# zcablii/SM3Det

Hardware: NVIDIA H100
Metric: backbone images/sec @1024^2 (fwd+bwd) (higher is better)
Workload: dtype f32 (bf16 hi+lo split operands on wgmma, fp32 accumulate; SIMT fp32 elsewhere)

## Files before the change

sm3det_b200/csrc/gemm_tc.cu:

```cuda
#define SM3_GEMM_KERNEL_IMPL
#include "gemm_tc.cuh"
#include <mutex>

namespace sm3 {
const char* last_error();
namespace gemm {

int pick_bn(int N) {
  static const int cand[] = {128, 96, 64, 32};
  for (int bn : cand)
    if (N % bn == 0) return bn;
  return 0;
}

static bool aligned16(const void* p) { return (reinterpret_cast<uintptr_t>(p) & 15u) == 0; }

long long packed_elems(int N, int K) {
  const long long kblocks = (K + BK - 1) / BK;
  return (long long)N * kblocks * BK * 2;
}

__global__ void __launch_bounds__(256) pack_b_kernel(const float* __restrict__ B, long long s_mn, long long s_k,
                                                    long long group_stride, int N, int K, int BN, uint16_t* __restrict__ out,
                                                    long long chunks_per_group) {
  const long long i = (long long)blockIdx.x * blockDim.x + threadIdx.x;
  if (i >= chunks_per_group) return;
  const int g = blockIdx.y;
  const int kblocks = (K + BK - 1) / BK;
  const int n = (int)(i % N);
  const long long r = i / N;
  const int c = (int)(r % 4), kb = (int)(r / 4);
  const float* src = B + (long long)g * group_stride + (long long)n * s_mn;
  uint32_t hi[4], lo[4];
#pragma unroll
  for (int e = 0; e < 8; e += 2) {
    float v[2];
#pragma unroll
    for (int q = 0; q < 2; ++q) {
      const int k = kb * BK + c * 8 + e + q;
      v[q] = (k < K) ? __ldg(src + (long long)k * s_k) : 0.f;
    }
    const uint32_t u0 = __float_as_uint(v[0]), u1 = __float_as_uint(v[1]);
    hi[e / 2] = __byte_perm(u0, u1, 0x7632);
    const uint32_t r0 = __float_as_uint(v[0] - __uint_as_float(u0 & 0xFFFF0000u)) + 0x8000u;
    const uint32_t r1 = __float_as_uint(v[1] - __uint_as_float(u1 & 0xFFFF0000u)) + 0x8000u;
    lo[e / 2] = __byte_perm(r0, r1, 0x7632);
  }
  const int nt = n / BN, row = n % BN;
  uint8_t* tile = reinterpret_cast<uint8_t*>(out + (long long)g * ((long long)N * kblocks * BK * 2)) +
                  ((long long)nt * kblocks + kb) * ((long long)BN * 128);
  const uint32_t o = kmajor_sw64_offset((uint32_t)row, (uint32_t)c);
  *reinterpret_cast<uint4*>(tile + o) = make_uint4(hi[0], hi[1], hi[2], hi[3]);
  *reinterpret_cast<uint4*>(tile + (long long)BN * 64 + o) = make_uint4(lo[0], lo[1], lo[2], lo[3]);
}

int pack_b(const float* B, long long s_mn, long long s_k, long long group_stride, int groups, int N, int K,
           uint16_t* out, cudaStream_t stream, int tile) {
  SM3_REQUIRE(B && out && N > 0 && K > 0 && groups >= 1, SM3_ERR_INVALID_ARG, "gemm pack: bad argument");
  const int BN = tile > 0 ? tile : pick_bn(N);
  SM3_REQUIRE(BN > 0 && BN % 8 == 0 && BN <= 256 && N % BN == 0, SM3_ERR_UNSUPPORTED_SHAPE, "gemm pack: N=%d has no tile width (tile=%d)", N, tile);
  SM3_REQUIRE((reinterpret_cast<uintptr_t>(out) & 15u) == 0, SM3_ERR_INVALID_ARG, "gemm pack: output must be 16B aligned");
  const long long kblocks = (K + BK - 1) / BK;
  const long long chunks = (long long)N * kblocks * 4;
  dim3 grid((unsigned)((chunks + 255) / 256), (unsigned)groups);
  pack_b_kernel<<<grid, 256, 0, stream>>>(B, s_mn, s_k, group_stride, N, K, BN, out, chunks);
  return check_launch("pack_b_kernel");
}

long long packed_act_elems(long long rows, int cols, int mn_major, int tile) {
  if (!mn_major) {
    const long long rt = (rows + tile - 1) / tile, kb = (cols + BK - 1) / BK;
    return rt * kb * 2 * (long long)tile * BK;
  }
  const long long ct = (cols + tile - 1) / tile, kb = (rows + BK - 1) / BK;
  return ct * kb * 2 * (long long)(plane_bytes(tile, true) / 2);
}

__global__ void __launch_bounds__(256) pack_act_k_kernel(const float* __restrict__ X, long long ld, const int* __restrict__ row_index,
                                                        long long rows, int K, int tile, uint16_t* __restrict__ out,
                                                        long long chunks) {
  const long long i = (long long)blockIdx.x * blockDim.x + threadIdx.x;
  if (i >= chunks) return;
  const int kblocks = (K + BK - 1) / BK;
  const int cpr = kblocks * 4;
  const long long row = i / cpr;
  const int cc = (int)(i % cpr), kb = cc >> 2, c = cc & 3;
  long long src_row = row < rows ? row : -1;
  if (src_row >= 0 && row_index) src_row = __ldg(row_index + row);
  float v[8];
#pragma unroll
  for (int e = 0; e < 8; ++e) v[e] = 0.f;
  if (src_row >= 0) {
    const int k = kb * BK + c * 8;
    const float* src = X + src_row * ld + k;
    if (k + 8 <= K) { const float4 a = ldg_f4(src), b = ldg_f4(src + 4); v[0] = a.x; v[1] = a.y; v[2] = a.z; v[3] = a.w; v[4] = b.x; v[5] = b.y; v[6] = b.z; v[7] = b.w; }
    else { for (int e = 0; e < 8; ++e) if (k + e < K) v[e] = __ldg(src + e); }
  }
  uint32_t hi[4], lo[4];
#pragma unroll
  for (int e = 0; e < 8; e += 2) {
    const uint32_t u0 = __float_as_uint(v[e]), u1 = __float_as_uint(v[e + 1]);
    hi[e / 2] = __byte_perm(u0, u1, 0x7632);
    const uint32_t r0 = __float_as_uint(v[e] - __uint_as_float(u0 & 0xFFFF0000u)) + 0x8000u;
    const uint32_t r1 = __float_as_uint(v[e + 1] - __uint_as_float(u1 & 0xFFFF0000u)) + 0x8000u;
    lo[e / 2] = __byte_perm(r0, r1, 0x7632);
  }
  const long long rt = row / tile; const int rr = (int)(row % tile);
  uint8_t* img = reinterpret_cast<uint8_t*>(out) + (rt * kblocks + kb) * ((long long)tile * 128);
  const uint32_t o = kmajor_sw64_offset((uint32_t)rr, (uint32_t)c);
  *reinterpret_cast<uint4*>(img + o) = make_uint4(hi[0], hi[1], hi[2], hi[3]);
  *reinterpret_cast<uint4*>(img + (long long)tile * 64 + o) = make_uint4(lo[0], lo[1], lo[2], lo[3]);
}

__global__ void __launch_bounds__(256) pack_act_mn_kernel(const float* __restrict__ X, long long ld, const int* __restrict__ row_index,
                                                         long long rows, int W, int tile, uint16_t* __restrict__ out,
                                                         long long chunks, long long rows_pad) {
  const long long i = (long long)blockIdx.x * blockDim.x + threadIdx.x;
  if (i >= chunks) return;
  const int ct = (W + tile - 1) / tile;
  const int cpr = ct * (tile / 8);
  const long long r = i / cpr;
  const int cc = (int)(i % cpr);
  const int mt = cc / (tile / 8), mc = cc % (tile / 8);
  const int col = mt * tile + mc * 8;
  long long src_row = r < rows ? r : -1;
  if (src_row >= 0 && row_index) src_row = __ldg(row_index + r);
  float4 a = make_float4(0.f, 0.f, 0.f, 0.f), b = a;
  if (src_row >= 0 && col + 8 <= W) { const float* src = X + src_row * ld + col; a = ldg_f4(src); b = ldg_f4(src + 4); }
  const float v[8] = {a.x, a.y, a.z, a.w, b.x, b.y, b.z, b.w};
  uint32_t hi[4], lo[4];
#pragma unroll
  for (int e = 0; e < 8; e += 2) {
    const uint32_t u0 = __float_as_uint(v[e]), u1 = __float_as_uint(v[e + 1]);
    hi[e / 2] = __byte_perm(u0, u1, 0x7632);
    const uint32_t r0 = __float_as_uint(v[e] - __uint_as_float(u0 & 0xFFFF0000u)) + 0x8000u;
    const uint32_t r1 = __float_as_uint(v[e + 1] - __uint_as_float(u1 & 0xFFFF0000u)) + 0x8000u;
    lo[e / 2] = __byte_perm(r0, r1, 0x7632);
  }
  const long long kblocks = rows_pad / BK;
  const long long kb = r / BK; const uint32_t k = (uint32_t)(r % BK);
  const uint32_t pb = plane_bytes(tile, true);
  uint8_t* img = reinterpret_cast<uint8_t*>(out) + ((long long)mt * kblocks + kb) * (2LL * pb);
  const uint32_t o = mnmajor_sw128_offset(k, (uint32_t)mc);
  *reinterpret_cast<uint4*>(img + o) = make_uint4(hi[0], hi[1], hi[2], hi[3]);
  *reinterpret_cast<uint4*>(img + pb + o) = make_uint4(lo[0], lo[1], lo[2], lo[3]);
}

int pack_act(const float* X, long long ld, const int* row_index, long long rows, int cols, int mn_major, int tile,
             uint16_t* out, cudaStream_t stream) {
  SM3_REQUIRE(X && out && rows > 0 && cols > 0, SM3_ERR_INVALID_ARG, "gemm pack_act: bad argument");
  SM3_REQUIRE(tile >= 32 && tile <= 256 && tile % 32 == 0, SM3_ERR_INVALID_ARG, "gemm pack_act: tile=%d", tile);
  SM3_REQUIRE(aligned16(X) && aligned16(out) && ld % 4 == 0 && cols % 4 == 0, SM3_ERR_INVALID_ARG, "gemm pack_act: alignment");
  if (!mn_major) {
    const long long rt = (rows + tile - 1) / tile, kb = (cols + BK - 1) / BK;
    const long long chunks = rt * tile * kb * 4;
    pack_act_k_kernel<<<(unsigned)((chunks + 255) / 256), 256, 0, stream>>>(X, ld, row_index, rows, cols, tile, out, chunks);
  } else {
    SM3_REQUIRE(cols % 8 == 0, SM3_ERR_UNSUPPORTED_SHAPE, "gemm pack_act: MN-major needs cols%%8==0");
    const long long rows_pad = (rows + BK - 1) / BK * BK;
    const long long ct = (cols + tile - 1) / tile;
    const long long chunks = rows_pad * ct * (tile / 8);
    pack_act_mn_kernel<<<(unsigned)((chunks + 255) / 256), 256, 0, stream>>>(X, ld, row_index, rows, cols, tile, out, chunks, rows_pad);
  }
  return check_launch("pack_act");
}

int launch(Params p, cudaStream_t stream) {
  if (p.b_packed && !p.B) p.B = reinterpret_cast<const float*>(p.b_packed);
  if (p.a_packed && !p.A) p.A = reinterpret_cast<const float*>(p.a_packed);
  SM3_REQUIRE(p.A && p.B && p.D, SM3_ERR_INVALID_ARG, "gemm: null operand");
  SM3_REQUIRE(p.M > 0 && p.N > 0 && p.K >= 0, SM3_ERR_INVALID_ARG, "gemm: bad shape %d %d %d", p.M, p.N, p.K);
  SM3_REQUIRE((p.a_smn == 1) != (p.a_sk == 1) || (p.a_smn == 1 && p.M == 1), SM3_ERR_INVALID_ARG,
              "gemm: A needs exactly one unit stride");
  const bool packed = p.b_packed != nullptr;
  const bool apacked = p.a_packed != nullptr;
  if (packed && !apacked) { p.b_smn = p.K; p.b_sk = 1; }
  if (apacked) {
    const bool amn = (p.a_smn == 1 && p.a_sk != 1);
    if (amn) { p.b_smn = 1; p.b_sk = p.N; } else { p.b_smn = p.K; p.b_sk = 1; }
  }
  SM3_REQUIRE((p.b_smn == 1) != (p.b_sk == 1), SM3_ERR_INVALID_ARG, "gemm: B needs exactly one unit stride");
  const bool a_mn = (p.a_smn == 1 && p.a_sk != 1), b_mn = (p.b_smn == 1 && p.b_sk != 1);
  if (p.BN == 0) p.BN = pick_bn(p.N);
  SM3_REQUIRE(p.BN >= 32 && p.BN <= MAX_BN && p.BN % 32 == 0 && p.N % p.BN == 0, SM3_ERR_UNSUPPORTED_SHAPE,
              "gemm: N=%d has no tile width (multiple of 32 <= 128 dividing N)", p.N);
  SM3_REQUIRE(aligned16(p.A) && aligned16(p.B) && aligned16(p.D), SM3_ERR_INVALID_ARG, "gemm: pointers must be 16B aligned");
  if (!a_mn) SM3_REQUIRE(p.a_smn % 4 == 0 && p.K % 4 == 0, SM3_ERR_UNSUPPORTED_SHAPE, "gemm: K-major A needs K%%4==0, lda%%4==0");
  else       SM3_REQUIRE(p.a_sk % 4 == 0 && p.M % 8 == 0, SM3_ERR_UNSUPPORTED_SHAPE, "gemm: MN-major A needs M%%8==0, lda%%4==0");
  if (!b_mn) SM3_REQUIRE(p.b_smn % 4 == 0 && p.K % 4 == 0, SM3_ERR_UNSUPPORTED_SHAPE, "gemm: K-major B needs K%%4==0, ldb%%4==0");
  else       SM3_REQUIRE(p.b_sk % 4 == 0, SM3_ERR_UNSUPPORTED_SHAPE, "gemm: MN-major B needs ldb%%4==0");
  SM3_REQUIRE(!(p.a_row_index && a_mn), SM3_ERR_INVALID_ARG, "gemm: row gather needs K-major A");
  SM3_REQUIRE(!(p.b_k_index && !b_mn), SM3_ERR_INVALID_ARG, "gemm: k gather needs MN-major B");
  SM3_REQUIRE(p.ldd % 4 == 0, SM3_ERR_UNSUPPORTED_SHAPE, "gemm: ldd%%4");
  if (p.epi & (EPI_GELU | EPI_AUXSTORE)) SM3_REQUIRE(!p.aux_out || (aligned16(p.aux_out) && p.ld_aux % 4 == 0), SM3_ERR_INVALID_ARG, "gemm: aux_out");
  if (p.epi & EPI_DGELU) SM3_REQUIRE(p.aux_in && aligned16(p.aux_in) && p.ld_aux % 4 == 0, SM3_ERR_INVALID_ARG, "gemm: aux_in");
  if (p.epi & EPI_BIAS) SM3_REQUIRE(p.bias && aligned16(p.bias) && p.bias_group_stride % 4 == 0, SM3_ERR_INVALID_ARG, "gemm: bias");
  if (p.epi & EPI_COLSCALE) SM3_REQUIRE(p.col_scale && aligned16(p.col_scale), SM3_ERR_INVALID_ARG, "gemm: col_scale");
  if (p.epi & EPI_ROWSCALE) SM3_REQUIRE(p.row_scale, SM3_ERR_INVALID_ARG, "gemm: row_scale");
  if (p.epi & EPI_COLSUM) SM3_REQUIRE(p.colsum && aligned16(p.colsum) && p.colsum_group_stride % 4 == 0, SM3_ERR_INVALID_ARG, "gemm: colsum");
  if (p.epi & EPI_RESID) SM3_REQUIRE(p.resid && aligned16(p.resid) && p.ld_resid % 4 == 0, SM3_ERR_INVALID_ARG, "gemm: resid");

  p.n_tiles = p.N / p.BN;
  p.m_tiles = (p.M + BM - 1) / BM;
  if (p.sched == SCHED_DENSE) {
    p.k_splits = 1; p.num_groups = 1;
    p.num_tiles = p.m_tiles * p.n_tiles;
  } else if (p.sched == SCHED_GROUPED) {
    SM3_REQUIRE(p.tile_group && p.num_m_tiles_dev, SM3_ERR_INVALID_ARG, "gemm: grouped schedule needs tile map");
    p.k_splits = 1;
    p.num_tiles = p.m_tiles * p.n_tiles;
  } else if (p.sched == SCHED_SPLITK) {
    SM3_REQUIRE(p.k_splits >= 1 && p.num_groups >= 1, SM3_ERR_INVALID_ARG, "gemm: split-K needs k_splits/num_groups");
    SM3_REQUIRE((p.epi & EPI_ATOMIC) || p.k_splits == 1, SM3_ERR_INVALID_ARG, "gemm: split-K>1 needs EPI_ATOMIC");
    p.num_tiles = p.num_groups * p.m_tiles * p.n_tiles * p.k_splits;
  } else {
    SM3_REQUIRE(false, SM3_ERR_INVALID_ARG, "gemm: bad schedule %d", p.sched);
  }
  {
    const long long a_ext = apacked ? 0 : a_mn ? (long long)p.K * p.a_sk : (long long)(p.a_row_index ? (1LL << 31) / (p.a_smn ? p.a_smn : 1) : p.M) * p.a_smn;
    const long long b_ext = packed ? 0 : b_mn ? (long long)(p.b_k_index ? 1 : p.K) * p.b_sk + p.N : (long long)p.N * p.b_smn;
    SM3_REQUIRE(a_ext < (1LL << 32) && b_ext < (1LL << 32), SM3_ERR_UNSUPPORTED_SHAPE, "gemm: operand larger than 2^32 elements");
  }
  p.nstages = STAGES; p.stage_bytes = STAGE_BYTES;
  if (apacked) {
    const unsigned sb = (16384u + 2u * plane_bytes(p.BN, b_mn) + 1023u) & ~1023u;
    int ns = (int)((unsigned)(STAGES * STAGE_BYTES) / sb);
    if (ns > MAX_STAGES) ns = MAX_STAGES;
    if (ns >= STAGES) { p.nstages = ns; p.stage_bytes = sb; }
  }
  int grid = persistent_grid_sms();
  if (grid > p.num_tiles) grid = p.num_tiles;
  if (grid < 1) grid = 1;
#define SM3_GEMM_LAUNCH_E(AMN, BMN, BPK, APK, EPIT)                                                                             \
  do {                                                                                                                          \
    cudaFuncSetAttribute(gemm_bf16x3_kernel<AMN, BMN, BPK, APK, EPIT>, cudaFuncAttributeMaxDynamicSharedMemorySize, (int)SMEM_BYTES); \
    gemm_bf16x3_kernel<AMN, BMN, BPK, APK, EPIT><<<grid, NUM_THREADS, SMEM_BYTES, stream>>>(p);                                     \
  } while (0)
#define SM3_GEMM_LAUNCH(AMN, BMN, BPK, APK) SM3_GEMM_LAUNCH_E(AMN, BMN, BPK, APK, -1)
  if (apacked) {
    SM3_REQUIRE(packed && a_mn == b_mn && p.BN == pick_bn(p.N) && !p.a_row_index && !p.b_k_index, SM3_ERR_INVALID_ARG,
                "gemm: packed A needs packed B of the same majorness (gathers are applied by the pack kernels)");
    SM3_REQUIRE(aligned16(p.a_packed) && aligned16(p.b_packed) && (p.b_packed_group_stride % 8) == 0, SM3_ERR_INVALID_ARG,
                "gemm: packed operands must be 16B aligned");
    constexpr int E_FFN2_TRAIN = EPI_BIAS | EPI_COLSCALE | EPI_RESID | EPI_AUXSTORE, E_FFN2_EVAL = EPI_BIAS | EPI_COLSCALE | EPI_RESID;
    if (a_mn) {
      if (p.epi == EPI_ATOMIC) SM3_GEMM_LAUNCH_E(true, true, true, true, EPI_ATOMIC);
      else if (p.epi == (EPI_ATOMIC | EPI_ROWSCALE)) SM3_GEMM_LAUNCH_E(true, true, true, true, EPI_ATOMIC | EPI_ROWSCALE);
      else SM3_GEMM_LAUNCH(true, true, true, true);
    } else {
      if (p.epi == 0) SM3_GEMM_LAUNCH_E(false, false, true, true, 0);
      else if (p.epi == EPI_BIAS) SM3_GEMM_LAUNCH_E(false, false, true, true, EPI_BIAS);
      else if (p.epi == E_FFN2_TRAIN) SM3_GEMM_LAUNCH_E(false, false, true, true, E_FFN2_TRAIN);
      else if (p.epi == E_FFN2_EVAL) SM3_GEMM_LAUNCH_E(false, false, true, true, E_FFN2_EVAL);
      else SM3_GEMM_LAUNCH(false, false, true, true);
    }
  }
  else if (packed) {
    SM3_REQUIRE(!a_mn && p.sched != SCHED_SPLITK && p.BN == pick_bn(p.N), SM3_ERR_INVALID_ARG,
                "gemm: packed B needs K-major A, a dense/grouped schedule and the default tile width");
    SM3_REQUIRE((reinterpret_cast<uintptr_t>(p.b_packed) & 15u) == 0 && (p.b_packed_group_stride % 8) == 0,
                SM3_ERR_INVALID_ARG, "gemm: packed B must be 16B aligned");
    SM3_GEMM_LAUNCH(false, false, true, false);
  }
  else if (!a_mn && !b_mn) SM3_GEMM_LAUNCH(false, false, false, false);
  else if (!a_mn && b_mn) SM3_GEMM_LAUNCH(false, true, false, false);
  else if (a_mn && b_mn) SM3_GEMM_LAUNCH(true, true, false, false);
  else SM3_REQUIRE(false, SM3_ERR_UNSUPPORTED_SHAPE, "gemm: MN-major A with K-major B is not instantiated");
#undef SM3_GEMM_LAUNCH_E
#undef SM3_GEMM_LAUNCH
  return check_launch("gemm_bf16x3_kernel");
}

}
}
```

sm3det_b200/csrc/gemm_tc.cuh:

```cuda
#pragma once
#include <type_traits>
#include "common.cuh"

namespace sm3 {
namespace gemm {

constexpr int BM = 128;
constexpr int BK = 32;
constexpr int MAX_BN = 128;
constexpr int STAGES = 6;
constexpr int NUM_CONS_WARPS = 8;
constexpr int NUM_PROD_WARPS = 8;
constexpr int FIRST_PROD_WARP = 8;
constexpr int NUM_THREADS = (NUM_CONS_WARPS + NUM_PROD_WARPS) * 32;
constexpr int CONS_REGS = 144, PROD_REGS = 112;
constexpr int MAX_UNITS = 4;

constexpr uint32_t OFF_A_HI = 0;
constexpr uint32_t OFF_A_LO = 8192;
constexpr uint32_t OFF_B_HI = 16384;
constexpr uint32_t OFF_B_LO = 24576;
constexpr uint32_t STAGE_BYTES = 32768;
constexpr uint32_t WG_A_BYTES = 4096;
constexpr int MAX_STAGES = 8;
constexpr uint32_t BAR_BYTES = 256;
constexpr int EPI_CW = 16;
constexpr uint32_t EPI_STAGE_ROW_FLOATS = EPI_CW + 4;
constexpr uint32_t EPI_STAGE_BYTES = 32 * EPI_STAGE_ROW_FLOATS * 4;
constexpr int MAX_EPI_WARPS = 8;
constexpr int COLSUM_SMEM_COLS = 3072;
constexpr uint32_t SMEM_BYTES = STAGES * STAGE_BYTES + BAR_BYTES + MAX_EPI_WARPS * EPI_STAGE_BYTES + COLSUM_SMEM_COLS * 4 + 1024;

enum Sched : int { SCHED_DENSE = 0, SCHED_GROUPED = 1, SCHED_SPLITK = 2 };

enum Epi : int {
  EPI_BIAS = 1,
  EPI_GELU = 2,
  EPI_DGELU = 4,
  EPI_COLSCALE = 8,
  EPI_ROWSCALE = 16,
  EPI_RESID = 32,
  EPI_ATOMIC = 64,
  EPI_AUXSTORE = 128,
  EPI_COLSUM = 256,
};

struct Params {
  const float* A; long long a_smn, a_sk;
  const float* B; long long b_smn, b_sk; long long b_group_stride;
  const int* a_row_index;
  const int* b_k_index;
  const uint16_t* b_packed; long long b_packed_group_stride;
  const uint16_t* a_packed;
  int M, N, K, BN;
  int sched;
  int num_tiles;
  int m_tiles, n_tiles, k_splits, num_groups;
  const int* tile_group;
  const int* num_m_tiles_dev;
  const int* seg_begin;
  const int* seg_end;
  float* D; long long ldd; long long d_group_stride;
  const float* bias; long long bias_group_stride;
  int epi;
  float* aux_out; const float* aux_in; long long ld_aux;
  const float* col_scale; const float* row_scale;
  const float* resid; long long ld_resid;
  float* colsum; long long colsum_group_stride;
  int passes;
  int nstages; unsigned stage_bytes;
  int debug;
};

__host__ __device__ inline uint32_t kmajor_sw64_offset(uint32_t row, uint32_t chunk) {
  return (row >> 3) * 512u + (row & 7u) * 64u + ((chunk ^ ((row >> 1) & 3u)) << 4);
}
__host__ __device__ inline uint32_t mnmajor_sw128_offset(uint32_t k, uint32_t mn_chunk ) {
  const uint32_t g = mn_chunk >> 3, cc = mn_chunk & 7u;
  return (g * 4u + (k >> 3)) * 1024u + (k & 7u) * 128u + ((cc ^ (k & 7u)) << 4);
}
constexpr uint32_t MN_LBO_BYTES = 4096;
constexpr uint32_t MN_SBO_BYTES = 1024;
constexpr uint32_t K_SBO_BYTES = 512;
__host__ __device__ inline uint32_t plane_bytes(int width, bool mn_major) {
  return mn_major ? (uint32_t)((width + 63) / 64) * 4096u : (uint32_t)width * 64u;
}

__host__ __device__ inline uint64_t make_smem_desc(uint32_t smem_addr, bool mn_major) {
  uint64_t d = 0;
  d |= (uint64_t)((smem_addr >> 4) & 0x3FFFu);
  if (mn_major) {
    d |= (uint64_t)((MN_LBO_BYTES >> 4) & 0x3FFFu) << 16;
    d |= (uint64_t)((MN_SBO_BYTES >> 4) & 0x3FFFu) << 32;
    d |= (uint64_t)1 << 62;
  } else {
    d |= (uint64_t)1 << 16;
    d |= (uint64_t)((K_SBO_BYTES >> 4) & 0x3FFFu) << 32;
    d |= (uint64_t)2 << 62;
  }
  return d;
}
#if defined(__CUDACC__) && defined(SM3_GEMM_KERNEL_IMPL)
}
}
#include "wgmma.cuh"
namespace sm3 {
namespace gemm {
__device__ __forceinline__ uint32_t smem_u32(const void* p) {
  return static_cast<uint32_t>(__cvta_generic_to_shared(p));
}
__device__ __forceinline__ void mbar_init(uint32_t bar, uint32_t count) {
  asm volatile("mbarrier.init.shared::cta.b64 [%0], %1;" ::"r"(bar), "r"(count) : "memory");
}
__device__ __forceinline__ void mbar_arrive(uint32_t bar) {
  asm volatile("mbarrier.arrive.shared::cta.b64 _, [%0];" ::"r"(bar) : "memory");
}
__device__ __forceinline__ bool mbar_try_wait(uint32_t bar, uint32_t parity) {
  uint32_t ok;
  asm volatile(
      "{\n\t.reg .pred p;\n\t"
      "mbarrier.try_wait.parity.shared::cta.b64 p, [%1], %2;\n\t"
      "selp.u32 %0, 1, 0, p;\n\t}"
      : "=r"(ok) : "r"(bar), "r"(parity) : "memory");
  return ok != 0;
}
__device__ __forceinline__ void mbar_wait(uint32_t bar, uint32_t parity) {
  if (mbar_try_wait(bar, parity)) return;
  const long long t0 = clock64();
  while (!mbar_try_wait(bar, parity)) {
    if (clock64() - t0 > 20000000000LL) __trap();
  }
}
__device__ __forceinline__ void fence_proxy_async_smem() {
  asm volatile("fence.proxy.async.shared::cta;" ::: "memory");
}
struct Tile {
  int m0, n0, group, k_begin, k_end;
  __device__ __forceinline__ int nkb() const { return (k_end - k_begin + BK - 1) / BK; }
};

__device__ __forceinline__ int total_tiles(const Params& p) {
  if (p.sched == SCHED_GROUPED) return __ldg(p.num_m_tiles_dev) * p.n_tiles;
  return p.num_tiles;
}

__device__ __forceinline__ Tile decode_tile(const Params& p, int t) {
  Tile tl;
  if (p.sched == SCHED_SPLITK) {
    const int s = t % p.k_splits;
    int rest = t / p.k_splits;
    const int nt = rest % p.n_tiles; rest /= p.n_tiles;
    const int mt = rest % p.m_tiles;
    tl.group = rest / p.m_tiles;
    tl.m0 = mt * BM; tl.n0 = nt * p.BN;
    int b = 0, e = p.K;
    if (p.seg_begin) { b = __ldg(p.seg_begin + tl.group); e = __ldg(p.seg_end + tl.group); }
    int len = e - b; if (len < 0) len = 0;
    int chunk = (len + p.k_splits - 1) / p.k_splits;
    chunk = (chunk + BK - 1) / BK * BK;
    tl.k_begin = b + s * chunk;
    tl.k_end = min(e, tl.k_begin + chunk);
    if (tl.k_end < tl.k_begin) tl.k_end = tl.k_begin;
  } else {
    const int mt = t / p.n_tiles, nt = t % p.n_tiles;
    tl.m0 = mt * BM; tl.n0 = nt * p.BN;
    tl.group = (p.sched == SCHED_GROUPED) ? __ldg(p.tile_group + mt) : 0;
    tl.k_begin = 0; tl.k_end = p.K;
  }
  return tl;
}

__device__ __forceinline__ void split4(const float4& x, uint32_t& h01, uint32_t& h23, uint32_t& l01,
                                       uint32_t& l23) {
  const uint32_t u0 = __float_as_uint(x.x), u1 = __float_as_uint(x.y);
  const uint32_t u2 = __float_as_uint(x.z), u3 = __float_as_uint(x.w);
  h01 = __byte_perm(u0, u1, 0x7632);
  h23 = __byte_perm(u2, u3, 0x7632);
  const uint32_t r0 = __float_as_uint(x.x - __uint_as_float(u0 & 0xFFFF0000u)) + 0x8000u;
  const uint32_t r1 = __float_as_uint(x.y - __uint_as_float(u1 & 0xFFFF0000u)) + 0x8000u;
  const uint32_t r2 = __float_as_uint(x.z - __uint_as_float(u2 & 0xFFFF0000u)) + 0x8000u;
  const uint32_t r3 = __float_as_uint(x.w - __uint_as_float(u3 & 0xFFFF0000u)) + 0x8000u;
  l01 = __byte_perm(r0, r1, 0x7632);
  l23 = __byte_perm(r2, r3, 0x7632);
}

template <bool A_MN, bool B_MN, bool B_PACKED, bool A_PACKED, int EPI_T>
__global__ void __launch_bounds__(NUM_THREADS, 1) gemm_bf16x3_kernel(const __grid_constant__ Params p) {
  const int EPI = (EPI_T >= 0) ? EPI_T : p.epi;
  extern __shared__ uint8_t smem_raw[];
  const uint32_t smem_base = (smem_u32(smem_raw) + 1023u) & ~1023u;
  const uint32_t bar_base = smem_base + STAGES * STAGE_BYTES;
  auto full_bar = [&](int s) { return bar_base + 8u * s; };
  auto empty_bar = [&](int s) { return bar_base + 64u + 8u * s; };
  const int NST = p.nstages;
  const uint32_t STB = p.stage_bytes;

  const int warp = threadIdx.x >> 5, lane = threadIdx.x & 31;

  if (threadIdx.x == 0) {
    for (int s = 0; s < NST; ++s) { mbar_init(full_bar(s), A_PACKED ? 1 : NUM_PROD_WARPS + (B_PACKED ? 1 : 0)); mbar_init(empty_bar(s), NUM_CONS_WARPS); }
    asm volatile("fence.mbarrier_init.release.cluster;" ::: "memory");
  }
  __syncthreads();

  const int ntiles = total_tiles(p);

  if (warp < NUM_CONS_WARPS) {
    asm volatile("setmaxnreg.inc.sync.aligned.u32 %0;" ::"n"(CONS_REGS));
    constexpr int NE = NUM_CONS_WARPS;
    const int wg = warp >> 2;
    const int nchunks = p.BN / EPI_CW;
    const uint32_t stage_base = bar_base + BAR_BYTES + (uint32_t)warp * EPI_STAGE_BYTES;
    const int rl = lane >> 2, c4 = (lane & 3) * 4;
    const uint32_t cs_base = bar_base + BAR_BYTES + MAX_EPI_WARPS * EPI_STAGE_BYTES;
    const bool cs_smem = (EPI & EPI_COLSUM) && p.N <= COLSUM_SMEM_COLS;
    int cs_group = -1;
    const int e_tid = warp * 32 + lane;
    auto epi_bar = []() { asm volatile("bar.sync 1, %0;" ::"n"(NE * 32) : "memory"); };
    auto cs_flush = [&](int group) {
      epi_bar();
      if (group >= 0) {
        float* cd = p.colsum + (long long)group * p.colsum_group_stride;
        for (int n = e_tid; n < p.N; n += NE * 32) {
          float sv;
          asm volatile("ld.shared.f32 %0, [%1];" : "=f"(sv) : "r"(cs_base + 4u * n) : "memory");
          if (sv != 0.f) atomicAdd(cd + n, sv);
        }
      }
      for (int n = e_tid; n < p.N; n += NE * 32)
        asm volatile("st.shared.f32 [%0], %1;" ::"r"(cs_base + 4u * n), "f"(0.f) : "memory");
      epi_bar();
    };
    if (cs_smem) cs_flush(-1);
    int stage = 0; uint32_t phase = 0;
    constexpr uint32_t a_kstep = A_MN ? 2u * MN_SBO_BYTES : 32u;
    constexpr uint32_t b_kstep = B_MN ? 2u * MN_SBO_BYTES : 32u;
    const uint32_t b_lo_off = B_PACKED ? OFF_B_HI + plane_bytes(p.BN, B_MN) : OFF_B_LO;
    float acc[MAX_BN / 2];
    for (int t = blockIdx.x; t < ntiles; t += gridDim.x) {
      const Tile tl = decode_tile(p, t);
      const int nkb = tl.nkb();
      if (nkb == 0) continue;
      if (cs_smem && tl.group != cs_group) { if (cs_group >= 0) cs_flush(cs_group); cs_group = tl.group; }
      const int row0 = tl.m0 + wg * 64 + (warp & 3) * 16;
      float4 rr[2], rn[2];
      auto load_resid = [&](int c_, float4 (&dst)[2]) {
        const int n_ = tl.n0 + c_ * EPI_CW + c4;
#pragma unroll
        for (int it = 0; it < 2; ++it) {
          const int row = row0 + it * 8 + rl;
          dst[it] = (row < p.M) ? ldg_f4(p.resid + (long long)row * p.ld_resid + n_) : make_float4(0.f, 0.f, 0.f, 0.f);
        }
      };
      if (EPI & EPI_RESID) load_resid(0, rr);

      int prev = -1;
      auto mainloop = [&](auto bn_c) {
        constexpr int N = decltype(bn_c)::value;
        for (int kb = 0; kb < nkb; ++kb) {
          mbar_wait(full_bar(stage), phase);
          wg::fence();
          const uint32_t sb = smem_base + stage * STB + (uint32_t)wg * WG_A_BYTES;
          const uint32_t sbb = smem_base + stage * STB;
#pragma unroll
          for (int j = 0; j < BK / 16; ++j) {
            const uint64_t ahi = make_smem_desc(sb + OFF_A_HI + j * a_kstep, A_MN);
            const uint64_t alo = make_smem_desc(sb + OFF_A_LO + j * a_kstep, A_MN);
            const uint64_t bhi = make_smem_desc(sbb + OFF_B_HI + j * b_kstep, B_MN);
            const uint64_t blo = make_smem_desc(sbb + b_lo_off + j * b_kstep, B_MN);
            if (!(p.debug & 4)) {
              const uint32_t accum = (kb > 0 || j > 0) ? 1u : 0u;
              if (p.passes == 1) {
                wg::mma<N, A_MN, B_MN>(acc, ahi, bhi, accum);
              } else {
                wg::mma<N, A_MN, B_MN>(acc, alo, bhi, accum);
                wg::mma<N, A_MN, B_MN>(acc, ahi, blo, 1u);
                wg::mma<N, A_MN, B_MN>(acc, ahi, bhi, 1u);
              }
            }
          }
          wg::commit();
          if (prev >= 0) {
            wg::wait<1>();
            __syncwarp();
            if (lane == 0) mbar_arrive(empty_bar(prev));
          }
          prev = stage;
          if (++stage == NST) { stage = 0; phase ^= 1u; }
        }
      };
      switch (p.BN) {
        case 32: mainloop(std::integral_constant<int, 32>{}); break;
        case 64: mainloop(std::integral_constant<int, 64>{}); break;
        case 96: mainloop(std::integral_constant<int, 96>{}); break;
        default: mainloop(std::integral_constant<int, 128>{}); break;
      }
      wg::wait<0>();
      wg::fence_operand(acc);
      __syncwarp();
      if (lane == 0) mbar_arrive(empty_bar(prev));
      if (p.debug & 4) {
#pragma unroll
        for (int i = 0; i < MAX_BN / 2; ++i) acc[i] = 0.f;
      }

      float* dbase = p.D + (long long)tl.group * p.d_group_stride;
      const float* bias = p.bias ? p.bias + (long long)tl.group * p.bias_group_stride : nullptr;
#pragma unroll
      for (int c = 0; c < MAX_BN / EPI_CW; ++c) {
        if (c >= nchunks) break;
        __syncwarp();
#pragma unroll
        for (int qq = 0; qq < 2; ++qq)
#pragma unroll
          for (int h = 0; h < 2; ++h)
            asm volatile("st.shared.v2.f32 [%0], {%1, %2};"
                         ::"r"(stage_base + (uint32_t)((rl + 8 * h) * EPI_STAGE_ROW_FLOATS + 8 * qq + 2 * (lane & 3)) * 4u),
                           "f"(acc[8 * c + 4 * qq + 2 * h]), "f"(acc[8 * c + 4 * qq + 2 * h + 1]) : "memory");
        if ((EPI & EPI_RESID) && c + 1 < nchunks) load_resid(c + 1, rn);
        __syncwarp();
        const int n = tl.n0 + c * EPI_CW + c4;
        float4 bv = make_float4(0.f, 0.f, 0.f, 0.f), sv = make_float4(1.f, 1.f, 1.f, 1.f);
        if (EPI & EPI_BIAS) bv = ldg_f4(bias + n);
        if (EPI & EPI_COLSCALE) sv = ldg_f4(p.col_scale + n);
        float4 cs = make_float4(0.f, 0.f, 0.f, 0.f);
#pragma unroll
        for (int it = 0; it < 2; ++it) {
          const int r = it * 8 + rl;
          const int row = row0 + r;
          if (row >= p.M) continue;
          float4 x;
          asm volatile("ld.shared.v4.f32 {%0, %1, %2, %3}, [%4];"
                       : "=f"(x.x), "=f"(x.y), "=f"(x.z), "=f"(x.w)
                       : "r"(stage_base + (uint32_t)(r * EPI_STAGE_ROW_FLOATS + c4) * 4u) : "memory");
          x.x += bv.x; x.y += bv.y; x.z += bv.z; x.w += bv.w;
          if ((EPI & (EPI_AUXSTORE | EPI_GELU)) && p.aux_out)
            *reinterpret_cast<float4*>(p.aux_out + (long long)row * p.ld_aux + n) = x;
          if (EPI & EPI_GELU) { x.x = gelu_fast(x.x); x.y = gelu_fast(x.y); x.z = gelu_fast(x.z); x.w = gelu_fast(x.w); }
          if (EPI & EPI_DGELU) {
            const float4 h = ldg_f4(p.aux_in + (long long)row * p.ld_aux + n);
            x.x *= gelu_grad_fast(h.x); x.y *= gelu_grad_fast(h.y); x.z *= gelu_grad_fast(h.z); x.w *= gelu_grad_fast(h.w);
          }
          x.x *= sv.x; x.y *= sv.y; x.z *= sv.z; x.w *= sv.w;
          if (EPI & EPI_ROWSCALE) { const float rs = __ldg(p.row_scale + row); x.x *= rs; x.y *= rs; x.z *= rs; x.w *= rs; }
          if (EPI & EPI_RESID) { x.x += rr[it].x; x.y += rr[it].y; x.z += rr[it].z; x.w += rr[it].w; }
          cs.x += x.x; cs.y += x.y; cs.z += x.z; cs.w += x.w;
          float* dst = dbase + (long long)row * p.ldd + n;
          if (EPI & EPI_ATOMIC) {
            asm volatile("red.global.add.v4.f32 [%0], {%1, %2, %3, %4};" ::"l"(dst), "f"(x.x), "f"(x.y), "f"(x.z), "f"(x.w) : "memory");
          } else {
            *reinterpret_cast<float4*>(dst) = x;
          }
        }
        if (EPI & EPI_RESID) {
#pragma unroll
          for (int it = 0; it < 2; ++it) rr[it] = rn[it];
        }
        if (EPI & EPI_COLSUM) {
#pragma unroll
          for (int o = 4; o < 32; o <<= 1) {
            cs.x += __shfl_xor_sync(0xffffffffu, cs.x, o); cs.y += __shfl_xor_sync(0xffffffffu, cs.y, o);
            cs.z += __shfl_xor_sync(0xffffffffu, cs.z, o); cs.w += __shfl_xor_sync(0xffffffffu, cs.w, o);
          }
          if (lane < 4) {
            if (cs_smem) {
              const uint32_t sa = cs_base + 4u * (uint32_t)n;
              asm volatile("red.shared.add.f32 [%0], %1;" ::"r"(sa), "f"(cs.x) : "memory");
              asm volatile("red.shared.add.f32 [%0], %1;" ::"r"(sa + 4u), "f"(cs.y) : "memory");
              asm volatile("red.shared.add.f32 [%0], %1;" ::"r"(sa + 8u), "f"(cs.z) : "memory");
              asm volatile("red.shared.add.f32 [%0], %1;" ::"r"(sa + 12u), "f"(cs.w) : "memory");
            } else {
              float* cd = p.colsum + (long long)tl.group * p.colsum_group_stride + n;
              asm volatile("red.global.add.v4.f32 [%0], {%1, %2, %3, %4};" ::"l"(cd), "f"(cs.x), "f"(cs.y), "f"(cs.z), "f"(cs.w) : "memory");
            }
          }
        }
      }
    }
    if (cs_smem && cs_group >= 0) cs_flush(cs_group);
  } else {
    asm volatile("setmaxnreg.dec.sync.aligned.u32 %0;" ::"n"(PROD_REGS));
    if (A_PACKED) {
      if (warp == FIRST_PROD_WARP && lane == 0) {
        const uint32_t a_bytes = 2u * plane_bytes(BM, A_MN), b_bytes = 2u * plane_bytes(p.BN, B_MN);
        const long long kblocks = (p.K + BK - 1) / BK;
        int stage = 0; uint32_t phase = 0;
        for (int t = blockIdx.x; t < ntiles; t += gridDim.x) {
          const Tile tl = decode_tile(p, t);
          const int nkb = tl.nkb();
          if (nkb == 0) continue;
          const long long kb0 = tl.k_begin / BK;
          const uint8_t* srcA = reinterpret_cast<const uint8_t*>(p.a_packed) + ((long long)(tl.m0 / BM) * kblocks + kb0) * a_bytes;
          const uint8_t* srcB = reinterpret_cast<const uint8_t*>(p.b_packed + (long long)tl.group * p.b_packed_group_stride) +
                                ((long long)(tl.n0 / p.BN) * kblocks + kb0) * b_bytes;
          for (int kb = 0; kb < nkb; ++kb) {
            mbar_wait(empty_bar(stage), phase ^ 1u);
            const uint32_t sb = smem_base + stage * STB;
            asm volatile("mbarrier.arrive.expect_tx.shared::cta.b64 _, [%0], %1;" ::"r"(full_bar(stage)), "r"(a_bytes + b_bytes) : "memory");
            asm volatile("cp.async.bulk.shared::cluster.global.mbarrier::complete_tx::bytes [%0], [%1], %2, [%3];"
                         ::"r"(sb + OFF_A_HI), "l"(srcA + (long long)kb * a_bytes), "r"(a_bytes), "r"(full_bar(stage)) : "memory");
            asm volatile("cp.async.bulk.shared::cluster.global.mbarrier::complete_tx::bytes [%0], [%1], %2, [%3];"
                         ::"r"(sb + OFF_B_HI), "l"(srcB + (long long)kb * b_bytes), "r"(b_bytes), "r"(full_bar(stage)) : "memory");
            if (++stage == NST) { stage = 0; phase ^= 1u; }
          }
        }
      }
    } else {
    const int wq = warp - FIRST_PROD_WARP;
    constexpr int units_a = 16;
    const int segs_b = (p.BN + 127) / 128;
    const int units_b = B_PACKED ? 0 : (B_MN ? 16 * segs_b : p.BN / 8);
    const int units = units_a + units_b;
    const uint32_t st_k = (uint32_t)((lane >> 2) * 64 + ((((uint32_t)lane & 3u) ^ (((uint32_t)lane >> 3) & 3u)) << 4));
    const uint32_t kr_lane = (uint32_t)lane >> 4, j_lane = (uint32_t)lane & 15u;

    constexpr int MU = B_PACKED ? (16 + NUM_PROD_WARPS - 1) / NUM_PROD_WARPS : MAX_UNITS;
    uint32_t off[MU];
    uint32_t vmask = 0;
    const float* baseB = p.B;
    const uint16_t* packB = nullptr;
    int t_cur = blockIdx.x - gridDim.x, kb_cur = 0, nkb_cur = 0, k_begin = 0, k_end = 0;
    const uint32_t adv_a = A_MN ? (uint32_t)(BK * p.a_sk) : (uint32_t)BK;
    const uint32_t adv_b = B_MN ? (uint32_t)(BK * p.b_sk) : (uint32_t)BK;
    const bool b_gather = B_MN && (p.b_k_index != nullptr);

    auto setup_tile = [&](const Tile& tl) {
      k_begin = tl.k_begin; k_end = tl.k_end;
      baseB = p.B + (long long)tl.group * p.b_group_stride;
      if (B_PACKED) {
        const long long kblocks = (p.K + BK - 1) / BK;
        packB = p.b_packed + (long long)tl.group * p.b_packed_group_stride +
                ((long long)(tl.n0 / p.BN) * kblocks) * (2LL * p.BN * BK);
      }
      vmask = 0;
#pragma unroll
      for (int i = 0; i < MU; ++i) {
        const int u = wq + NUM_PROD_WARPS * i;
        off[i] = 0;
        if (u >= units) continue;
        const bool is_a = u < units_a;
        const int ul = is_a ? u : u - units_a;
        const int mn0 = is_a ? tl.m0 : tl.n0;
        const int mn_lim = is_a ? p.M : p.N;
        if (is_a ? !A_MN : !B_MN) {
          const long long s_mn = is_a ? p.a_smn : p.b_smn;
          const int row = mn0 + 8 * ul + (lane >> 2);
          if (row >= mn_lim) continue;
          long long ridx = row;
          if (is_a && p.a_row_index) { ridx = __ldg(p.a_row_index + row); if (ridx < 0) continue; }
          off[i] = (uint32_t)(ridx * s_mn + tl.k_begin + 8 * (lane & 3));
          vmask |= 1u << i;
        } else {
          const int segs = is_a ? 1 : segs_b;
          const int pi = (segs == 2) ? (ul >> 1) : ul, seg = (segs == 2) ? (ul & 1) : 0;
          const int mnl = seg * 128 + 8 * (int)j_lane;
          const int tile_w = is_a ? BM : p.BN;
          if (mnl + 8 > tile_w || mn0 + mnl + 8 > mn_lim) continue;
          const long long s_k = is_a ? p.a_sk : p.b_sk;
          const int koff = 2 * pi + (int)kr_lane;
          off[i] = (!is_a && b_gather) ? (uint32_t)(mn0 + mnl)
                                       : (uint32_t)((long long)(tl.k_begin + koff) * s_k + mn0 + mnl);
          vmask |= 1u << i;
        }
      }
    };
    auto advance = [&]() -> bool {
      if (kb_cur + 1 < nkb_cur) { ++kb_cur; return true; }
      for (t_cur += gridDim.x; t_cur < ntiles; t_cur += gridDim.x) {
        const Tile tl = decode_tile(p, t_cur);
        nkb_cur = tl.nkb();
        if (nkb_cur > 0) { kb_cur = 0; setup_tile(tl); return true; }
      }
      return false;
    };

    auto load_kb = [&](float4 (&r)[MU][2]) {
      const int k0 = k_begin + kb_cur * BK;
      const int kl = k0 + 8 * (lane & 3);
      const bool kin0 = (kl + 4 <= k_end), kin1 = (kl + 8 <= k_end);
#pragma unroll
      for (int i = 0; i < MU; ++i) {
        r[i][0] = make_float4(0.f, 0.f, 0.f, 0.f);
        r[i][1] = make_float4(0.f, 0.f, 0.f, 0.f);
        const int u = wq + NUM_PROD_WARPS * i;
        if (u >= units) continue;
        const bool is_a = u < units_a;
        const float* base = is_a ? p.A : baseB;
        const bool ok = (vmask >> i) & 1u;
        if (is_a ? !A_MN : !B_MN) {
          if (ok && kin0) r[i][0] = ldg_f4(base + off[i]);
          if (ok && kin1) r[i][1] = ldg_f4(base + off[i] + 4);
        } else {
          const int ul = is_a ? u : u - units_a;
          const int pi = (!is_a && segs_b == 2) ? (ul >> 1) : ul;
          const int k = k0 + 2 * pi + (int)kr_lane;
          if (ok && k < k_end) {
            const float* src = base + off[i];
            if (!is_a && b_gather) {
              const int kk = __ldg(p.b_k_index + k);
              src = (kk >= 0) ? base + (long long)kk * p.b_sk + off[i] : nullptr;
            }
            if (src) { r[i][0] = ldg_f4(src); r[i][1] = ldg_f4(src + 4); }
          }
        }
        off[i] += is_a ? adv_a : ((!is_a && b_gather) ? 0u : adv_b);
      }
    };

    auto store_kb = [&](const float4 (&r)[MU][2], uint32_t sb) {
#pragma unroll
      for (int i = 0; i < MU; ++i) {
        const int u = wq + NUM_PROD_WARPS * i;
        if (u >= units) continue;
        const bool is_a = u < units_a;
        const int ul = is_a ? u : u - units_a;
        uint4 hi, lo;
        split4(r[i][0], hi.x, hi.y, lo.x, lo.y);
        split4(r[i][1], hi.z, hi.w, lo.z, lo.w);
        uint32_t o;
        if (is_a ? !A_MN : !B_MN) {
          o = (uint32_t)ul * 512u + st_k;
        } else {
          const int segs = is_a ? 1 : segs_b;
          const uint32_t pi = (segs == 2) ? (uint32_t)(ul >> 1) : (uint32_t)ul;
          const uint32_t seg = (segs == 2) ? (uint32_t)(ul & 1) : 0u;
          const uint32_t k = 2u * pi + kr_lane;
          const uint32_t mc = seg * 16u + j_lane;
          o = ((mc >> 3) * 4u + (k >> 3)) * 1024u + (k & 7u) * 128u + (((mc & 7u) ^ (k & 7u)) << 4);
        }
        const uint32_t dst_hi = sb + (is_a ? OFF_A_HI : OFF_B_HI) + o;
        const uint32_t dst_lo = sb + (is_a ? OFF_A_LO : OFF_B_LO) + o;
        asm volatile("st.shared.v4.b32 [%0], {%1, %2, %3, %4};"
                     ::"r"(dst_hi), "r"(hi.x), "r"(hi.y), "r"(hi.z), "r"(hi.w) : "memory");
        asm volatile("st.shared.v4.b32 [%0], {%1, %2, %3, %4};"
                     ::"r"(dst_lo), "r"(lo.x), "r"(lo.y), "r"(lo.z), "r"(lo.w) : "memory");
      }
    };

    int stage = 0; uint32_t phase = 0;
    const uint16_t* pub_src = nullptr; int pub_kb = 0;
    auto publish = [&](const float4 (&r)[MU][2]) {
      mbar_wait(empty_bar(stage), phase ^ 1u);
      if (B_PACKED && wq == 0 && lane == 0 && (p.debug & 2)) {
        mbar_arrive(full_bar(stage));
      } else if (B_PACKED && wq == 0 && lane == 0) {
        const uint32_t bytes = (uint32_t)p.BN * 128u;
        const uint16_t* src = pub_src + (long long)pub_kb * (2LL * p.BN * BK);
        asm volatile("mbarrier.arrive.expect_tx.shared::cta.b64 _, [%0], %1;" ::"r"(full_bar(stage)), "r"(bytes) : "memory");
        asm volatile("cp.async.bulk.shared::cluster.global.mbarrier::complete_tx::bytes [%0], [%1], %2, [%3];"
                     ::"r"(smem_base + stage * STB + OFF_B_HI), "l"(src), "r"(bytes), "r"(full_bar(stage)) : "memory");
      }
      if (p.debug & 8) {
#pragma unroll
        for (int i = 0; i < MU; ++i) asm volatile("" ::"f"(r[i][0].x), "f"(r[i][1].w));
      } else if (!(p.debug & 1)) store_kb(r, smem_base + stage * STB);
      fence_proxy_async_smem();
      __syncwarp();
      if (lane == 0) mbar_arrive(full_bar(stage));
      if (++stage == NST) { stage = 0; phase ^= 1u; }
    };

    constexpr int PF = B_PACKED ? 4 : 2;
    float4 r[PF][MU][2];
    if (p.debug & 16) {
#pragma unroll
      for (int d = 0; d < PF; ++d)
#pragma unroll
        for (int i = 0; i < MU; ++i) { r[d][i][0] = make_float4(1.f, 2.f, 3.f, 4.f); r[d][i][1] = r[d][i][0]; }
    }
    const uint16_t* q_src[PF]; int q_kb[PF]; bool q_ok[PF];
    const bool dbg_noload = p.debug & (1 | 16);
#pragma unroll
    for (int d = 0; d < PF; ++d) {
      q_ok[d] = advance();
      q_src[d] = packB; q_kb[d] = kb_cur;
      if (q_ok[d] && !dbg_noload) load_kb(r[d]);
    }
    bool done = !q_ok[0];
    while (!done) {
#pragma unroll
      for (int d = 0; d < PF; ++d) {
        if (!q_ok[d]) { done = true; break; }
        pub_src = q_src[d]; pub_kb = q_kb[d];
        publish(r[d]);
        q_ok[d] = advance();
        q_src[d] = packB; q_kb[d] = kb_cur;
        if (q_ok[d] && !dbg_noload) load_kb(r[d]);
      }
    }
    }
  }

}
#endif

long long packed_elems(int N, int K);
int pack_b(const float* B, long long s_mn, long long s_k, long long group_stride, int groups, int N, int K,
           uint16_t* out, cudaStream_t stream, int tile = 0);
long long packed_act_elems(long long rows, int cols, int mn_major, int tile);
int pack_act(const float* X, long long ld, const int* row_index, long long rows, int cols, int mn_major, int tile,
             uint16_t* out, cudaStream_t stream);
int launch(Params p, cudaStream_t stream);
int pick_bn(int N);

}
}
```

Measured before the change: 79.26.

## Offload packed-A GEMM epilogue to idle producer warps via smem accumulator buffer

For K-major fully packed GEMMs, the seven producer warps left idle by the single-thread bulk-copy producer become dedicated epilogue warps. Consumers dump accumulators into a swizzled shared-memory buffer guarded by full/empty mbarriers, then move straight to the next tile's mainloop while the epilogue warps apply bias, GELU, scaling, residual, colsum and stores. This overlaps epilogue work with the next tile's MMA. In exchange the accumulator buffer takes ring space and cuts pipeline stages, and the new path errors if fewer than four stages fit.

```diff
diff --git a/sm3det_b200/csrc/gemm_tc.cu b/sm3det_b200/csrc/gemm_tc.cu
--- a/sm3det_b200/csrc/gemm_tc.cu
+++ b/sm3det_b200/csrc/gemm_tc.cu
@@ -221,12 +221,15 @@
     const long long b_ext = packed ? 0 : b_mn ? (long long)(p.b_k_index ? 1 : p.K) * p.b_sk + p.N : (long long)p.N * p.b_smn;
     SM3_REQUIRE(a_ext < (1LL << 32) && b_ext < (1LL << 32), SM3_ERR_UNSUPPORTED_SHAPE, "gemm: operand larger than 2^32 elements");
   }
-  p.nstages = STAGES; p.stage_bytes = STAGE_BYTES;
+  p.nstages = STAGES; p.stage_bytes = STAGE_BYTES; p.epi_warps = 0;
   if (apacked) {
     const unsigned sb = (16384u + 2u * plane_bytes(p.BN, b_mn) + 1023u) & ~1023u;
-    int ns = (int)((unsigned)(STAGES * STAGE_BYTES) / sb);
+    p.epi_warps = use_epilogue_warps(a_mn, true) && p.K >= MIN_EPI_WARPS_K;
+    const unsigned acc = p.epi_warps ? acc_buf_bytes(p.BN) : 0u;
+    int ns = (int)((unsigned)(STAGES * STAGE_BYTES - acc) / sb);
     if (ns > MAX_STAGES) ns = MAX_STAGES;
-    if (ns >= STAGES) { p.nstages = ns; p.stage_bytes = sb; }
+    SM3_REQUIRE(ns >= MIN_PACKED_STAGES, SM3_ERR_UNSUPPORTED_SHAPE, "gemm: fully packed ring of %d stages at BN=%d", ns, p.BN);
+    p.nstages = ns; p.stage_bytes = sb;
   }
   int grid = persistent_grid_sms();
   if (grid > p.num_tiles) grid = p.num_tiles;
diff --git a/sm3det_b200/csrc/gemm_tc.cuh b/sm3det_b200/csrc/gemm_tc.cuh
--- a/sm3det_b200/csrc/gemm_tc.cuh
+++ b/sm3det_b200/csrc/gemm_tc.cuh
@@ -30,6 +30,11 @@
 constexpr int MAX_EPI_WARPS = 8;
 constexpr int COLSUM_SMEM_COLS = 3072;
 constexpr uint32_t SMEM_BYTES = STAGES * STAGE_BYTES + BAR_BYTES + MAX_EPI_WARPS * EPI_STAGE_BYTES + COLSUM_SMEM_COLS * 4 + 1024;
+constexpr int NUM_EPI_WARPS = NUM_PROD_WARPS - 1;
+constexpr int MIN_PACKED_STAGES = 4;
+__host__ __device__ constexpr bool use_epilogue_warps(bool a_mn, bool a_packed) { return a_packed && !a_mn; }
+constexpr int MIN_EPI_WARPS_K = 64;
+__host__ __device__ constexpr uint32_t acc_buf_bytes(int bn) { return (uint32_t)BM * (uint32_t)bn * 4u; }
 
 enum Sched : int { SCHED_DENSE = 0, SCHED_GROUPED = 1, SCHED_SPLITK = 2 };
 
@@ -69,6 +74,7 @@
   float* colsum; long long colsum_group_stride;
   int passes;
   int nstages; unsigned stage_bytes;
+  int epi_warps;
   int debug;
 };
 
@@ -184,14 +190,101 @@
   l23 = __byte_perm(r2, r3, 0x7632);
 }
 
+__device__ __forceinline__ void load_resid_block(const Params& p, int row0, int n, int rl, float4 (&dst)[2]) {
+#pragma unroll
+  for (int it = 0; it < 2; ++it) {
+    const int row = row0 + it * 8 + rl;
+    dst[it] = (row < p.M) ? ldg_f4(p.resid + (long long)row * p.ld_resid + n) : make_float4(0.f, 0.f, 0.f, 0.f);
+  }
+}
+
+__device__ __forceinline__ void epilogue_block(const Params& p, const int EPI, float* dbase, const float* bias, int group,
+                                               int row0, int n, const uint32_t (&x_addr)[2], const float4 (&rr)[2],
+                                               bool cs_smem, uint32_t cs_base, int lane) {
+  const int rl = lane >> 2;
+  float4 bv = make_float4(0.f, 0.f, 0.f, 0.f), sv = make_float4(1.f, 1.f, 1.f, 1.f);
+  if (EPI & EPI_BIAS) bv = ldg_f4(bias + n);
+  if (EPI & EPI_COLSCALE) sv = ldg_f4(p.col_scale + n);
+  float4 cs = make_float4(0.f, 0.f, 0.f, 0.f);
+#pragma unroll
+  for (int it = 0; it < 2; ++it) {
+    const int row = row0 + it * 8 + rl;
+    if (row >= p.M) continue;
+    float4 x;
+    asm volatile("ld.shared.v4.f32 {%0, %1, %2, %3}, [%4];"
+                 : "=f"(x.x), "=f"(x.y), "=f"(x.z), "=f"(x.w) : "r"(x_addr[it]) : "memory");
+    x.x += bv.x; x.y += bv.y; x.z += bv.z; x.w += bv.w;
+    if ((EPI & (EPI_AUXSTORE | EPI_GELU)) && p.aux_out)
+      *reinterpret_cast<float4*>(p.aux_out + (long long)row * p.ld_aux + n) = x;
+    if (EPI & EPI_GELU) { x.x = gelu_fast(x.x); x.y = gelu_fast(x.y); x.z = gelu_fast(x.z); x.w = gelu_fast(x.w); }
+    if (EPI & EPI_DGELU) {
+      const float4 h = ldg_f4(p.aux_in + (long long)row * p.ld_aux + n);
+      x.x *= gelu_grad_fast(h.x); x.y *= gelu_grad_fast(h.y); x.z *= gelu_grad_fast(h.z); x.w *= gelu_grad_fast(h.w);
+    }
+    x.x *= sv.x; x.y *= sv.y; x.z *= sv.z; x.w *= sv.w;
+    if (EPI & EPI_ROWSCALE) { const float rs = __ldg(p.row_scale + row); x.x *= rs; x.y *= rs; x.z *= rs; x.w *= rs; }
+    if (EPI & EPI_RESID) { x.x += rr[it].x; x.y += rr[it].y; x.z += rr[it].z; x.w += rr[it].w; }
+    cs.x += x.x; cs.y += x.y; cs.z += x.z; cs.w += x.w;
+    float* dst = dbase + (long long)row * p.ldd + n;
+    if (EPI & EPI_ATOMIC) {
+      asm volatile("red.global.add.v4.f32 [%0], {%1, %2, %3, %4};" ::"l"(dst), "f"(x.x), "f"(x.y), "f"(x.z), "f"(x.w) : "memory");
+    } else {
+      *reinterpret_cast<float4*>(dst) = x;
+    }
+  }
+  if (EPI & EPI_COLSUM) {
+#pragma unroll
+    for (int o = 4; o < 32; o <<= 1) {
+      cs.x += __shfl_xor_sync(0xffffffffu, cs.x, o); cs.y += __shfl_xor_sync(0xffffffffu, cs.y, o);
+      cs.z += __shfl_xor_sync(0xffffffffu, cs.z, o); cs.w += __shfl_xor_sync(0xffffffffu, cs.w, o);
+    }
+    if (lane < 4) {
+      if (cs_smem) {
+        const uint32_t sa = cs_base + 4u * (uint32_t)n;
+        asm volatile("red.shared.add.f32 [%0], %1;" ::"r"(sa), "f"(cs.x) : "memory");
+        asm volatile("red.shared.add.f32 [%0], %1;" ::"r"(sa + 4u), "f"(cs.y) : "memory");
+        asm volatile("red.shared.add.f32 [%0], %1;" ::"r"(sa + 8u), "f"(cs.z) : "memory");
+        asm volatile("red.shared.add.f32 [%0], %1;" ::"r"(sa + 12u), "f"(cs.w) : "memory");
+      } else {
+        float* cd = p.colsum + (long long)group * p.colsum_group_stride + n;
+        asm volatile("red.global.add.v4.f32 [%0], {%1, %2, %3, %4};" ::"l"(cd), "f"(cs.x), "f"(cs.y), "f"(cs.z), "f"(cs.w) : "memory");
+      }
+    }
+  }
+}
+
+template <int NT>
+__device__ __forceinline__ void colsum_flush(const Params& p, uint32_t cs_base, int group, int e_tid) {
+  asm volatile("bar.sync 1, %0;" ::"n"(NT) : "memory");
+  if (group >= 0) {
+    float* cd = p.colsum + (long long)group * p.colsum_group_stride;
+    for (int n = e_tid; n < p.N; n += NT) {
+      float sv;
+      asm volatile("ld.shared.f32 %0, [%1];" : "=f"(sv) : "r"(cs_base + 4u * n) : "memory");
+      if (sv != 0.f) atomicAdd(cd + n, sv);
+    }
+  }
+  for (int n = e_tid; n < p.N; n += NT)
+    asm volatile("st.shared.f32 [%0], %1;" ::"r"(cs_base + 4u * n), "f"(0.f) : "memory");
+  asm volatile("bar.sync 1, %0;" ::"n"(NT) : "memory");
+}
+
+__device__ __forceinline__ uint32_t acc_buf_offset(uint32_t row, uint32_t granule, uint32_t bn) {
+  return row * bn * 4u + ((granule ^ (((row & 1u) << 2) | (row & 2u))) << 4);
+}
+
 template <bool A_MN, bool B_MN, bool B_PACKED, bool A_PACKED, int EPI_T>
 __global__ void __launch_bounds__(NUM_THREADS, 1) gemm_bf16x3_kernel(const __grid_constant__ Params p) {
   const int EPI = (EPI_T >= 0) ? EPI_T : p.epi;
+  constexpr bool EPI_WARPS = use_epilogue_warps(A_MN, A_PACKED);
+  const bool epi_warps = EPI_WARPS && p.epi_warps;
   extern __shared__ uint8_t smem_raw[];
   const uint32_t smem_base = (smem_u32(smem_raw) + 1023u) & ~1023u;
   const uint32_t bar_base = smem_base + STAGES * STAGE_BYTES;
   auto full_bar = [&](int s) { return bar_base + 8u * s; };
   auto empty_bar = [&](int s) { return bar_base + 64u + 8u * s; };
+  const uint32_t acc_full = bar_base + 128u, acc_empty = bar_base + 136u;
+  const uint32_t acc_base = bar_base - acc_buf_bytes(p.BN);
   const int NST = p.nstages;
   const uint32_t STB = p.stage_bytes;
 
@@ -199,6 +292,7 @@
 
   if (threadIdx.x == 0) {
     for (int s = 0; s < NST; ++s) { mbar_init(full_bar(s), A_PACKED ? 1 : NUM_PROD_WARPS + (B_PACKED ? 1 : 0)); mbar_init(empty_bar(s), NUM_CONS_WARPS); }
+    if (epi_warps) { mbar_init(acc_full, NUM_CONS_WARPS * 32); mbar_init(acc_empty, NUM_EPI_WARPS * 32); }
     asm volatile("fence.mbarrier_init.release.cluster;" ::: "memory");
   }
   __syncthreads();
@@ -231,7 +325,8 @@
         asm volatile("st.shared.f32 [%0], %1;" ::"r"(cs_base + 4u * n), "f"(0.f) : "memory");
       epi_bar();
     };
-    if (cs_smem) cs_flush(-1);
+    if (!epi_warps && cs_smem) cs_flush(-1);
+    uint32_t acc_phase = 0;
     int stage = 0; uint32_t phase = 0;
     constexpr uint32_t a_kstep = A_MN ? 2u * MN_SBO_BYTES : 32u;
     constexpr uint32_t b_kstep = B_MN ? 2u * MN_SBO_BYTES : 32u;
@@ -241,7 +336,7 @@
       const Tile tl = decode_tile(p, t);
       const int nkb = tl.nkb();
       if (nkb == 0) continue;
-      if (cs_smem && tl.group != cs_group) { if (cs_group >= 0) cs_flush(cs_group); cs_group = tl.group; }
+      if (!epi_warps && cs_smem && tl.group != cs_group) { if (cs_group >= 0) cs_flush(cs_group); cs_group = tl.group; }
       const int row0 = tl.m0 + wg * 64 + (warp & 3) * 16;
       float4 rr[2], rn[2];
       auto load_resid = [&](int c_, float4 (&dst)[2]) {
@@ -252,7 +347,7 @@
           dst[it] = (row < p.M) ? ldg_f4(p.resid + (long long)row * p.ld_resid + n_) : make_float4(0.f, 0.f, 0.f, 0.f);
         }
       };
-      if (EPI & EPI_RESID) load_resid(0, rr);
+      if (!epi_warps && (EPI & EPI_RESID)) load_resid(0, rr);
 
       int prev = -1;
       auto mainloop = [&](auto bn_c) {
@@ -304,6 +399,23 @@
         for (int i = 0; i < MAX_BN / 2; ++i) acc[i] = 0.f;
       }
 
+      if (epi_warps) {
+        mbar_wait(acc_empty, acc_phase ^ 1u);
+        const uint32_t r_frag = (uint32_t)(wg * 64 + (warp & 3) * 16 + rl);
+#pragma unroll
+        for (int q = 0; q < MAX_BN / 8; ++q) {
+          if (q >= p.BN / 8) break;
+#pragma unroll
+          for (int h = 0; h < 2; ++h)
+            asm volatile("st.shared.v2.f32 [%0], {%1, %2};"
+                         ::"r"(acc_base + acc_buf_offset(r_frag + 8u * h, 2u * q + ((lane & 3) >> 1), p.BN) + (lane & 1) * 8u),
+                           "f"(acc[4 * q + 2 * h]), "f"(acc[4 * q + 2 * h + 1]) : "memory");
+        }
+        mbar_arrive(acc_full);
+        acc_phase ^= 1u;
+        continue;
+      }
+
       float* dbase = p.D + (long long)tl.group * p.d_group_stride;
       const float* bias = p.bias ? p.bias + (long long)tl.group * p.bias_group_stride : nullptr;
 #pragma unroll
@@ -377,10 +489,56 @@
         }
       }
     }
-    if (cs_smem && cs_group >= 0) cs_flush(cs_group);
+    if (!epi_warps && cs_smem && cs_group >= 0) cs_flush(cs_group);
   } else {
     asm volatile("setmaxnreg.dec.sync.aligned.u32 %0;" ::"n"(PROD_REGS));
-    if (A_PACKED) {
+    if (EPI_WARPS && warp > FIRST_PROD_WARP) {
+      if (!epi_warps) return;
+      const int rl = lane >> 2, c4 = (lane & 3) * 4;
+      const int nchunks = p.BN / EPI_CW;
+      const uint32_t cs_base = bar_base + BAR_BYTES + MAX_EPI_WARPS * EPI_STAGE_BYTES;
+      const bool cs_smem = (EPI & EPI_COLSUM) && p.N <= COLSUM_SMEM_COLS;
+      const int ew = warp - FIRST_PROD_WARP - 1;
+      constexpr int NT = NUM_EPI_WARPS * 32;
+      const int e_tid = ew * 32 + lane;
+      const int nblocks = (BM / 16) * nchunks;
+      int cs_group = -1;
+      if (cs_smem) colsum_flush<NT>(p, cs_base, -1, e_tid);
+      uint32_t acc_phase = 0;
+      for (int t = blockIdx.x; t < ntiles; t += gridDim.x) {
+        const Tile tl = decode_tile(p, t);
+        if (tl.nkb() == 0) continue;
+        if (cs_smem && tl.group != cs_group) {
+          if (cs_group >= 0) colsum_flush<NT>(p, cs_base, cs_group, e_tid);
+          cs_group = tl.group;
+        }
+        float* dbase = p.D + (long long)tl.group * p.d_group_stride;
+        const float* bias = p.bias ? p.bias + (long long)tl.group * p.bias_group_stride : nullptr;
+        float4 rr[2], rn[2];
+        if ((EPI & EPI_RESID) && ew < nblocks)
+          load_resid_block(p, tl.m0 + (ew / nchunks) * 16, tl.n0 + (ew % nchunks) * EPI_CW + c4, rl, rr);
+        mbar_wait(acc_full, acc_phase);
+        for (int i = ew; i < nblocks; i += NUM_EPI_WARPS) {
+          const int rg = i / nchunks, c = i % nchunks;
+          if ((EPI & EPI_RESID) && i + NUM_EPI_WARPS < nblocks) {
+            const int j = i + NUM_EPI_WARPS;
+            load_resid_block(p, tl.m0 + (j / nchunks) * 16, tl.n0 + (j % nchunks) * EPI_CW + c4, rl, rn);
+          }
+          const uint32_t g = (uint32_t)(c * (EPI_CW / 4) + (lane & 3));
+          const uint32_t x_addr[2] = {acc_base + acc_buf_offset((uint32_t)(rg * 16 + rl), g, p.BN),
+                                      acc_base + acc_buf_offset((uint32_t)(rg * 16 + 8 + rl), g, p.BN)};
+          epilogue_block(p, EPI, dbase, bias, tl.group, tl.m0 + rg * 16, tl.n0 + c * EPI_CW + c4, x_addr, rr, cs_smem,
+                         cs_base, lane);
+          if (EPI & EPI_RESID) {
+#pragma unroll
+            for (int it = 0; it < 2; ++it) rr[it] = rn[it];
+          }
+        }
+        mbar_arrive(acc_empty);
+        acc_phase ^= 1u;
+      }
+      if (cs_smem && cs_group >= 0) colsum_flush<NT>(p, cs_base, cs_group, e_tid);
+    } else if (A_PACKED) {
       if (warp == FIRST_PROD_WARP && lane == 0) {
         const uint32_t a_bytes = 2u * plane_bytes(BM, A_MN), b_bytes = 2u * plane_bytes(p.BN, B_MN);
         const long long kblocks = (p.K + BK - 1) / BK;
```

Result: faster. 80.24 (median of 6 runs) (+1.2%).
